# tjamescouch/abnn

Hardware: AMD Instinct MI355X
Metric: traversal events/sec at 1B synapses, 5M neurons; achieved HBM GB/s (higher is better)
Workload: dtype f32

## Files before the change

### abnn_amd/_lib.py

```python
from __future__ import annotations

import ctypes as C
import os

_HERE = os.path.dirname(os.path.abspath(__file__))
LIB_PATH = os.environ.get("ABNN_LIB") or os.path.join(_HERE, "libabnn_hip.so")

SUMMARY_WORDS = 4
COMM_ID_BYTES = 128


class Dims(C.Structure):

    _fields_ = [
        ("n_input", C.c_uint32),
        ("n_output", C.c_uint32),
        ("n_hidden", C.c_uint64),
        ("n_syn", C.c_uint64),
        ("events_per_pass", C.c_uint64),
        ("syn_offset", C.c_uint64),
        ("global_events", C.c_uint64),
        ("syn_capacity", C.c_uint64),
    ]

# ... 471 lines not shown
                   "abnn_reorder_host",
                   "abnn_propagate_words", "abnn_propagate_enqueue", "abnn_propagate", "abnn_propagate_rescale_enqueue",
                   "abnn_propagate_iterate_enqueue", "abnn_propagate_host", "abnn_propagate_rescale_host")

_lib = None


def _share_hip_runtime_with_torch() -> None:
    import importlib.util

    spec = importlib.util.find_spec("torch")
    if spec is None or not spec.submodule_search_locations:
        return
    hip = os.path.join(list(spec.submodule_search_locations)[0], "lib", "libamdhip64.so")
    if os.path.exists(hip):
        C.CDLL(hip, mode=C.RTLD_GLOBAL)


DEBUG_SIGNATURES = [
    ("abnn_debug_set_wave_clock", C.c_int, [_VP, C.c_int]),
    ("abnn_debug_raw_stats", C.c_int, [_VP, C.POINTER(C.c_uint64), _VP]),
    ("abnn_debug_raw_gate_timing", C.c_int, [C.c_int]),
    ("abnn_debug_raw_gate_time", C.c_int, [C.POINTER(C.c_double), _PU32]),
    ("abnn_debug_raw_fused", C.c_int, [C.c_int]),
    ("abnn_debug_raw_fused_active", C.c_int, []),
    ("abnn_debug_raw_wave_clock", C.c_int, [_VP, C.c_uint64, _U32, _U32, C.POINTER(C.c_uint64), C.c_uint64, _VP]),
    ("abnn_debug_live_allocations", C.c_uint64, []),
    ("abnn_debug_set_propagate_path", C.c_int, [_VP, C.c_int]),
    ("abnn_debug_index_state", C.c_int, [_VP, C.POINTER(C.c_uint64), C.POINTER(C.c_double)]),
    ("abnn_debug_index_mask_dirty", C.c_int, [_VP, C.POINTER(C.c_uint64)]),
    ("abnn_debug_set_indexed", C.c_int, [_VP, C.c_int]),
    ("abnn_debug_set_fused", C.c_int, [_VP, C.c_int]),
    ("abnn_debug_index_copy", C.c_int, [_VP, _PU32, C.c_uint64, _PU32, C.c_uint64]),
]


def load() -> C.CDLL:
    global _lib
    if _lib is not None:
        return _lib
    if not os.path.exists(LIB_PATH):
        raise ImportError(
            f"{LIB_PATH} not found: build it with `python -c 'import __graft_entry__ as g; g.build()'` "
            "(there is no CPU fallback for the traversal engine)")
    _share_hip_runtime_with_torch()
    lib = C.CDLL(LIB_PATH)
    for name, res, args in SIGNATURES + DEBUG_SIGNATURES:
        if not hasattr(lib, name) and ((name, res, args) in DEBUG_SIGNATURES or
                                       (os.environ.get("ABNN_LIB") and name in ABI10_ADDITIONS)):
            continue
        fn = getattr(lib, name)
        fn.restype = res
        fn.argtypes = args
    got = lib.abnn_abi_version()
    if got != ABI_VERSION:
        if not os.environ.get("ABNN_LIB_ANY_ABI"):
            raise ImportError(f"{LIB_PATH}: ABI version {got}, this binding is {ABI_VERSION} "
                              "(ABNN_LIB_ANY_ABI=1 accepts it for pass timing only)")
        import warnings

        warnings.warn(f"{LIB_PATH}: ABI version {got} != {ABI_VERSION}; use pass/timing entry points only")
    _lib = lib
    return lib


def check(fn_name: str, status: int) -> None:
# ... 24 lines not shown
```

### abnn_amd/csrc/capi.hip

```cpp
#include <dlfcn.h>
#include <link.h>
#include <rccl/rccl.h>

#include <algorithm>
#include <chrono>
#include <condition_variable>
#include <cstdio>
#include <cstdlib>
#include <cstring>
#include <mutex>
#include <new>
#include <string>
#include <vector>

#include "census.h"
#include "degree.h"
#include "select.h"
#include "edit.h"
#include "snapshot.h"
#include "graph.h"
#include "hops.h"
#include "engine.h"
#include "learn.h"
#include "spikes.h"
// ... 13 lines not shown
namespace {

#define HIP_TRY(expr)                                                                  \
    do {                                                                               \
        hipError_t _e = (expr);                                                        \
        if (_e != hipSuccess) {                                                        \
            set_err(std::string(#expr) + ": " + hipGetErrorString(_e));                \
            return ABNN_ERR_HIP;                                                       \
        }                                                                              \
    } while (0)

#define REQUIRE(cond, msg)                                                             \
    do {                                                                               \
        if (!(cond)) {                                                                 \
            set_err(msg);                                                              \
            return ABNN_ERR_INVALID;                                                   \
        }                                                                              \
    } while (0)

uint64_t visited_events(const abnn_dims& d, uint32_t mode)
{
    if (mode == ABNN_MODE_RANDOM) return d.n_syn ? d.events_per_pass : 0;
    uint64_t grid = (d.events_per_pass + 255u) / 256u * 256u;
    return grid < d.n_syn ? grid : d.n_syn;
}

struct EventPair {
    hipEvent_t a, b;
};

struct IndexState {
    uint32_t *row = nullptr, *off = nullptr, *mask = nullptr, *info = nullptr;
    uint4* heavy = nullptr;
    uint32_t heavy_chunks = 0;
    uint64_t mask_words = 0;
    bool built = false;
    uint64_t entries = 0;
    uint32_t max_degree = 0;
    float build_ms = 0.0f;
    uint64_t eligible = 0;
    bool last_indexed = false;
    uint64_t indexed_passes = 0;
    int flavour = -1;
    int mode = 1;
    uint32_t after = 4;
    uint64_t max_mb = 4096;
};

}

struct abnn_brain {
    abnn_dims dims{};
    abnn_params params{};
    KernelParams kp{};
    int device = 0;
    hipStream_t stream = nullptr;
    uint64_t n_nrn = 0;
    DevicePool pool;
    DeviceState d{};
    void* scalar_block = nullptr;
    uint64_t clock_host = 0;
    uint64_t rng = 0;
    uint64_t stim_first = 0, stim_count = 0;
    uint64_t clean_passes = 0, max_host_stamp = 0;
    uint64_t stim_ring[kFiredRing][2] = {};
    bool next_built = false;
// ... 210 lines not shown
void host_tick(abnn_brain* b)
{
    if (tick_events(b) > 0) b->clock_host += b->params.clock_inc;
}

abnn_status time_begin(abnn_brain* b, hipStream_t s, EventPair** out)
{
    *out = nullptr;
    if (b->timing <= 0) return ABNN_OK;
    const uint64_t n = (uint64_t)b->timing, c = b->timing_count++;
    if (c % n != (n > 1 ? 1u : 0u)) return ABNN_OK;
    if (b->events_used == b->events.size()) {
        EventPair p;
        HIP_TRY(hipEventCreate(&p.a));
        HIP_TRY(hipEventCreate(&p.b));
        b->events.push_back(p);
    }
    *out = &b->events[b->events_used++];
    HIP_TRY(hipEventRecord((*out)->a, s));
    return ABNN_OK;
}

constexpr uint64_t kStreamPinMiB = 160;
uint64_t stream_pin_bytes()
{
    uint64_t mib = kStreamPinMiB;
    if (const char* env = std::getenv("ABNN_STREAM_PIN_MB")) mib = (uint64_t)std::min(4096, std::max(0, std::atoi(env)));
    return mib << 20;
}

void index_invalidate(abnn_brain* b)
{
    IndexState& x = b->ix;
    if (x.row || x.off || x.mask || x.info || x.heavy) {
        (void)hipSetDevice(b->device);
        b->pool.release(&x.row, &x.off, &x.mask, &x.info, &x.heavy);
    }
    x.heavy_chunks = 0;
    x.built = false;
    x.entries = 0;
    x.max_degree = 0;
    x.mask_words = 0;
    x.eligible = 0;
}

void configure(abnn_brain* b)
{
    DeviceState& d = b->d;
    d.n_syn = b->dims.n_syn;
    const uint64_t ev = visited_events(b->dims, b->params.mode);
    if (ev != d.events) index_invalidate(b);
    d.events = ev;
    const uint64_t iters = (d.events + d.iter_events - 1) / d.iter_events;
    d.iters = (uint32_t)iters;
    uint64_t G = std::min<uint64_t>(iters, std::min<uint64_t>((uint64_t)b->cus * b->per_cu, kMaxGateBlocks));
    const uint64_t waves = d.gate_block / 64;
    G = std::min<uint64_t>(G, (iters + waves - 1) / waves);
    if (G == 0 && iters > 0) G = 1;
    d.gate_blocks = (uint32_t)G;
    d.n_ranges = (uint32_t)(G * waves);
    const uint64_t budget = stream_pin_bytes();
    d.pin_k = 0;
    if (d.events > 0 && b->params.mode == ABNN_MODE_SWEEP && !b->params.track_visits)
        d.pin_k = (uint32_t)std::min<uint64_t>(16, 16 * budget / (3 * d.events));
}

abnn_status reset_ranges(abnn_brain* b)
{
    const DeviceState& d = b->d;
    std::vector<uint32_t> rb(d.n_ranges + 1);
// ... 138 lines not shown
    d.stim_first = b->stim_first;
    d.stim_count = b->stim_count;
    const bool prebuilt = b->next_built && b->built_stim[0] == b->stim_first &&
                          b->built_stim[1] == b->stim_count;
    b->next_built = false;
    if (was_prebuilt) *was_prebuilt = prebuilt;
    if (!prebuilt) HIP_TRY(launch_bitmap(d, b->kp, b->stim_first, b->stim_count, s));
    b->stim_ring[b->pass_host % kFiredRing][0] = b->stim_first;
    b->stim_ring[b->pass_host % kFiredRing][1] = b->stim_count;
    return ABNN_OK;
}

void plan_build(abnn_brain* b)
{
    DeviceState& d = b->d;
    d.build_next = build_next_ok(b) ? 1u : 0u;
    d.n_next_stim = 0;
    if (d.build_next) {
        const uint64_t W = b->params.window_pre, p = b->pass_host;
        auto add = [&](uint64_t f, uint64_t c) {
            if (c == 0) return;
            for (uint32_t r = 0; r < d.n_next_stim; ++r)
                if (d.next_stim[r][0] == f && d.next_stim[r][1] == c) return;
            d.next_stim[d.n_next_stim][0] = f;
            d.next_stim[d.n_next_stim++][1] = c;
        };
        for (uint64_t q = p + 1 - W; q <= p; ++q) add(b->stim_ring[q % kFiredRing][0], b->stim_ring[q % kFiredRing][1]);
        add(b->stim_first, b->stim_count);
    }
}

uint64_t index_bytes(const abnn_brain* b)
{
    return 4 * b->d.events + 4 * (b->n_nrn + 1) + 4 * index_mask_words(b->d.iters, b->d.iter_events);
}

bool index_eligible(const abnn_brain* b)
{
    const DeviceState& d = b->d;
    const abnn_params& p = b->params;
    const bool plastic = p.w_prune > 0.0f || (d.grown != nullptr && p.p_new > 0.0f);
    return b->ix.mode != 0 && p.mode == ABNN_MODE_SWEEP && !p.track_visits && !plastic && d.lean && !d.g2src &&
           !b->ext_ptrs && b->dims.global_events == 0 && d.events > 0 && d.events < (1ull << 32) &&
           index_bytes(b) <= (b->ix.max_mb << 20);
}

bool index_pass_rule(const abnn_brain* b, bool prebuilt)
{
    if (!prebuilt) return false;
    const uint64_t W = b->params.window_pre, p = b->pass_host;
    uint64_t stim = b->stim_count;
    for (uint64_t q = p >= W ? p - W : 0; q <= p; ++q) stim = std::max(stim, b->stim_ring[q % kFiredRing][1]);
    const uint64_t bound = W * ((uint64_t)b->params.max_spikes + stim);
    return bound * b->ix.max_degree <= b->d.events / 8;
}

abnn_status index_build(abnn_brain* b, hipStream_t s)
{
    IndexState& x = b->ix;
    const DeviceState& d = b->d;
    index_invalidate(b);
    DeviceTemp<uint32_t> cursor, part;
    x.mask_words = index_mask_words(d.iters, d.iter_events);
    abnn_status st = b->pool.alloc_all({raw(&x.row, b->n_nrn + 1), raw(&x.off, d.events), zeroed(&x.mask, x.mask_words),
                                        zeroed(&x.info, 4)});
    if (st == ABNN_OK) st = cursor.alloc(b->n_nrn + 1, false);
    if (st == ABNN_OK) st = part.alloc(index_tiles(b->n_nrn) + 1, false);
    if (st != ABNN_OK) {
        index_invalidate(b);
        x.mode = 0;
        return st == ABNN_ERR_OOM ? ABNN_OK : st;
    }
    hipEvent_t ea = nullptr, eb = nullptr;
    HIP_TRY(hipEventCreate(&ea));
    hipError_t e = hipEventCreate(&eb);
    uint32_t info[4] = {0, 0, 0, 0};
    float ms = 0.0f;
    if (e == hipSuccess) e = hipEventRecord(ea, s);
    if (e == hipSuccess) e = launch_index_build(d.syn, d.events, b->n_nrn, x.row, cursor.dev, part.dev, x.off, x.info, (uint32_t)b->cus, s);
    if (e == hipSuccess) e = hipEventRecord(eb, s);
    if (e == hipSuccess) e = hipMemcpyAsync(info, x.info, sizeof(info), hipMemcpyDeviceToHost, s);
    if (e == hipSuccess) e = hipStreamSynchronize(s);
    if (e == hipSuccess) e = hipEventElapsedTime(&ms, ea, eb);
    (void)hipEventDestroy(ea);
    if (eb) (void)hipEventDestroy(eb);
    HIP_TRY(e);
    x.max_degree = info[0];
    x.entries = info[1];
    x.build_ms = ms;
    if (info[2]) {
        st = b->pool.alloc(raw(&x.heavy, info[2]));
        if (st != ABNN_OK) {
            index_invalidate(b);
            x.mode = 0;
            return st == ABNN_ERR_OOM ? ABNN_OK : st;
        }
        HIP_TRY(launch_index_heavy(x.row, b->n_nrn, x.heavy, info[2], x.info, s));
    }
// ... 43 lines not shown
        b->next_built = d.build_next != 0;
        b->built_stim[0] = b->stim_first;
        b->built_stim[1] = b->stim_count;
        rotate_bounds(b);
        return ABNN_OK;
    }
    plan_build(b);
    HIP_TRY(launch_apply(d, b->kp, gathered, world, rank, s));
    b->next_built = d.build_next != 0;
    b->built_stim[0] = b->stim_first;
    b->built_stim[1] = b->stim_count;
    rotate_bounds(b);
    return ABNN_OK;
}

abnn_status run_fused(abnn_brain* b, hipStream_t s)
{
    DeviceState& d = b->d;
    IndexState& x = b->ix;
    const bool eligible = index_eligible(b);
    if (eligible && !x.built && x.eligible >= x.after) ST_TRY(index_build(b, s));
    bool prebuilt = false;
    ST_TRY(pass_buffers(b, s, &prebuilt));
    plan_build(b);
    const bool indexed = eligible && x.built && (x.mode == 2 || index_pass_rule(b, prebuilt));
    d.prologue_adapt = b->last_pass_fused && x.flavour == (indexed ? 1 : 0) && d.adapt_ranges ? 1u : 0u;
    d.cost_in = b->cost_buf[b->cost_parity ^ 1u];
    d.cost_out = b->cost_buf[b->cost_parity];
    d.indexed = indexed ? 1u : 0u;
    d.ev_mask = x.mask;
    EventPair* ev = nullptr;
    ST_TRY(time_begin(b, s, &ev));
    hipError_t e = hipSuccess;
    if (indexed)
        e = launch_index_mark(d.bitmap, d.n_bitmap_words, d.n_nrn, x.row, x.off, x.mask, d.events, x.heavy, x.heavy_chunks, s);
    if (e == hipSuccess) e = launch_fused_pass(d, b->kp, s);
    d.indexed = 0u;
    HIP_TRY(e);
    if (ev) HIP_TRY(hipEventRecord(ev->b, s));
    x.flavour = indexed ? 1 : 0;
    x.last_indexed = indexed;
    x.indexed_passes += indexed ? 1u : 0u;
    x.eligible = eligible ? x.eligible + 1 : 0;
    b->next_built = d.build_next != 0;
    b->built_stim[0] = b->stim_first;
    b->built_stim[1] = b->stim_count;
    rotate_bounds(b);
    b->cost_parity ^= 1u;
    b->last_pass_fused = true;
    return ABNN_OK;
}

abnn_status run_shard_fused_gate(abnn_brain* b, int32_t* xchg, hipStream_t s)
{
    DeviceState& d = b->d;
    ST_TRY(pass_buffers(b, s));
    plan_build(b);
    d.prologue_adapt = b->last_pass_fused && d.adapt_ranges ? 1u : 0u;
    d.cost_in = b->cost_buf[b->cost_parity ^ 1u];
    d.cost_out = b->cost_buf[b->cost_parity];
    d.shard_mode = 1;
    d.xchg = xchg;
    b->ix.eligible = 0;
    b->ix.last_indexed = false;
    b->ix.flavour = 0;
    EventPair* ev = nullptr;
    ST_TRY(time_begin(b, s, &ev));
    const hipError_t e = launch_fused_pass(d, b->kp, s);
// ... 1979 lines not shown
    ST_TRY(sync_all(b));
    HIP_TRY(hipMemcpy(out, b->d.range_bounds, std::min<uint64_t>(n, b->d.n_ranges + 1ull) * 4, hipMemcpyDeviceToHost));
    return ABNN_OK;
}

abnn_status abnn_debug_stream_pin(abnn_brain* b, uint32_t* pin_k)
{
    REQUIRE(b && pin_k, "null argument");
    *pin_k = b->d.pin_k;
    return ABNN_OK;
}

abnn_status abnn_debug_index_state(abnn_brain* b, uint64_t out[ABNN_DEBUG_INDEX_WORDS], double* build_ms)
{
    REQUIRE(b && out, "null argument");
    const IndexState& x = b->ix;
    out[0] = x.built ? 1 : 0;
    out[1] = x.entries;
    out[2] = x.max_degree;
    out[3] = x.last_indexed ? 1 : 0;
    out[4] = x.indexed_passes;
    out[5] = x.eligible;
    out[6] = (uint64_t)x.mode;
    out[7] = b->d.events;
    if (build_ms) *build_ms = x.build_ms;
    return ABNN_OK;
}

abnn_status abnn_debug_index_mask_dirty(abnn_brain* b, uint64_t* words)
{
    REQUIRE(b && words, "null argument");
    *words = 0;
    ST_TRY(sync_all(b));
    if (!b->ix.mask) return ABNN_OK;
    HIP_TRY(launch_index_dirty(b->ix.mask, b->ix.mask_words, reinterpret_cast<unsigned long long*>(b->u64_scratch), b->stream));
    return read_words(b, b->u64_scratch, words, 1);
}

abnn_status abnn_debug_set_indexed(abnn_brain* b, int mode)
{
    REQUIRE(b && mode >= 0 && mode <= 2, "abnn_debug_set_indexed: mode must be 0, 1 or 2");
    b->ix.mode = mode;
    return ABNN_OK;
}

abnn_status abnn_debug_set_fused(abnn_brain* b, int on)
{
    REQUIRE(b, "null argument");
    REQUIRE(!b->pending_walk, "abnn_debug_set_fused: a sharded pass is half done (abnn_shard_apply)");
    b->use_fused = on != 0;
    return ABNN_OK;
}

abnn_status abnn_debug_index_copy(abnn_brain* b, uint32_t* row, uint64_t n_row, uint32_t* off, uint64_t n_off)
{
    REQUIRE(b && (row || n_row == 0) && (off || n_off == 0), "null argument");
    ST_TRY(sync_all(b));
    REQUIRE(b->ix.built, "abnn_debug_index_copy: no index is built");
    REQUIRE(n_row <= b->n_nrn + 1 && n_off <= b->ix.entries, "abnn_debug_index_copy: range out of bounds");
    if (n_row) HIP_TRY(hipMemcpy(row, b->ix.row, n_row * 4, hipMemcpyDeviceToHost));
    if (n_off) HIP_TRY(hipMemcpy(off, b->ix.off, n_off * 4, hipMemcpyDeviceToHost));
    return ABNN_OK;
}

uint64_t abnn_debug_live_allocations(void) { return g_live_allocations.load(std::memory_order_relaxed); }

abnn_status abnn_get_stats(abnn_brain* b, abnn_stats* out)
{
    REQUIRE(b && out, "null argument");
// ... 545 lines not shown
```

### abnn_amd/csrc/engine.h

```cpp
#pragma once

#include <hip/hip_runtime.h>
#include <cstdint>

#include "../../include/abnn/abnn.h"

namespace abnn {

constexpr int kMaxFilterWords = 16384;
constexpr uint32_t kF2Words = 2048;
__host__ __device__ inline uint32_t f2_hash1(uint32_t n) { return (n * 0x9E3779B1u) >> 16; }
__host__ __device__ inline uint32_t f2_hash2(uint32_t n) { return (n * 0x85EBCA77u + 0x165667B1u) >> 16; }
constexpr int kScanThreads = 1024;
constexpr int kMaxGateBlocks = 1024;
constexpr int kMaxRanges = 16384;
constexpr int kApplyThreads = 1024;
constexpr uint32_t kCandCap = 256;
constexpr uint32_t kFusedMaxRanges = 4096;
constexpr uint32_t kWalkBlocks = 256;
constexpr int kMaxApplyBlocks = kWalkBlocks;
static_assert(kMaxApplyBlocks <= kApplyThreads, "the finalizing workgroup reads one apply partial per thread");
static_assert(kMaxRanges % kApplyThreads == 0, "range prefix: whole ranges per thread");
constexpr int kDummyRecords = 64 * 32;
constexpr uint32_t kFiredRing = 8;
// ... 95 lines not shown
    uint32_t chunk_penalty;
    uint32_t apply_blocks;
    uint32_t range_map;
    uint32_t pin_k;
    uint64_t* lb_status;
    const uint32_t* cost_in;
    uint32_t* cost_out;
    uint2* cand_list;
    uint32_t flush_at;
    int32_t spec_margin;
    uint32_t spec_mode;
    uint32_t lean;
    uint32_t shard_mode;
    int32_t* xchg;
    uint32_t prologue_adapt;
    uint64_t n_syn;
    uint64_t n_nrn;
    uint32_t n_input;
    uint64_t events;
    uint64_t syn_offset;
    uint64_t seed;
    uint32_t mode;
    uint32_t n_bitmap_words;
    uint32_t filter_words;
    uint32_t filter_log2;
    uint32_t gate_blocks;
    uint32_t n_ranges;
    uint32_t iters;
    uint32_t iter_events;
    uint32_t gate_block;
    uint32_t gate_k;
    uint32_t fused_max_blocks;
    uint32_t indexed;
    uint32_t* ev_mask;
};

struct KernelParams {
    float base_scale, target_rate_hz, eta_home, eta_reward, alpha_rbar;
    float a_ltp, a_ltd, w_min, w_max;
    uint32_t refractory, window_pre, clock_inc, max_spikes;
    uint32_t track_visits;
    float w_prune, p_new, w_init;
    uint32_t compact_every;
};

__host__ __device__ constexpr uint32_t xchg_words(uint32_t max_spikes)
{
    return 2 * ABNN_SUMMARY_WORDS + ((max_spikes + 1u) & ~1u);
}

constexpr int kCompactThreads = 1024;
constexpr int kCompactChunk = 4 * kCompactThreads;

KernelParams to_kernel_params(const abnn_params& p);

bool gate_shape_supported(uint32_t block, uint32_t k, uint32_t filter_words);
int gate_blocks_per_cu(uint32_t block, uint32_t k, uint32_t filter_words, bool track, bool random);

hipError_t launch_bitmap(const DeviceState& d, const KernelParams& kp, uint64_t stim_first,
                         uint64_t stim_count, hipStream_t s);
hipError_t launch_gate(const DeviceState& d, const KernelParams& kp, hipStream_t s);
bool fused_pass_supported(const DeviceState& d);
int fused_blocks_per_cu(uint32_t block, uint32_t k, uint32_t filter_words, bool track);
hipError_t launch_fused_pass(const DeviceState& d, const KernelParams& kp, hipStream_t s);
hipError_t launch_shard_walk(const DeviceState& d, const KernelParams& kp, const int32_t* gathered, uint32_t world,
                             uint32_t rank, hipStream_t s);
hipError_t launch_scan(const DeviceState& d, const KernelParams& kp, int32_t* xchg_out, hipStream_t s);
// ... 22 lines not shown
```

### abnn_amd/csrc/index.h

```cpp
#pragma once

#include "engine.h"

namespace abnn {

constexpr uint32_t kMaskRoundBytes = 4096;
inline uint64_t index_mask_words(uint64_t iters, uint64_t iter_events)
{
    return iters * iter_events / 32 + 2 * kMaskRoundBytes / 4;
}

constexpr uint32_t kIndexTile = 4096;
inline uint64_t index_tiles(uint64_t n_nrn) { return (n_nrn + kIndexTile - 1) / kIndexTile; }

hipError_t launch_index_build(const SynArrays& syn, uint64_t events, uint64_t n_nrn, uint32_t* row, uint32_t* cursor,
                              uint32_t* part, uint32_t* off, uint32_t* info, uint32_t cus, hipStream_t s);
hipError_t launch_index_heavy(const uint32_t* row, uint64_t n_nrn, uint4* heavy, uint32_t chunks, uint32_t* info,
                              hipStream_t s);
hipError_t launch_index_mark(const uint32_t* bitmap, uint32_t n_words, uint64_t n_nrn, const uint32_t* row,
                             const uint32_t* off, uint32_t* mask, uint64_t events, const uint4* heavy, uint32_t chunks,
                             hipStream_t s);
hipError_t launch_index_dirty(const uint32_t* mask, uint64_t words, unsigned long long* out, hipStream_t s);

}
```

### abnn_amd/csrc/index.hip

```cpp
#include "index.h"
#include "runs.h"
#include "scan.h"
#include "device.h"

namespace abnn {
namespace {

constexpr uint32_t kHeavyLen = 128, kHeavyChunk = 1024;

__device__ __forceinline__ void wave_lds_sync()
{
    __builtin_amdgcn_fence(__ATOMIC_RELEASE, "wavefront", "local");
    __builtin_amdgcn_wave_barrier();
    __builtin_amdgcn_fence(__ATOMIC_ACQUIRE, "wavefront", "local");
}

struct SrcPair {
    uint32_t k0, k1;
};

__device__ __forceinline__ SrcPair load_src_pair(const SynArrays& a, uint64_t base, uint32_t lane, uint64_t events,
                                                 uint32_t n_nrn)
{
    const uint64_t p = (base >> 1) + lane;
// ... 83 lines not shown
    }
    uint32_t total;
    uint32_t ex = part[blockIdx.x] + block_scan_u32(sum, &total, s_wave);
#pragma unroll
    for (uint32_t j = 0; j < 4; ++j) {
        if (i0 + j < n_nrn) {
            row[i0 + j] = ex;
            cursor[i0 + j] = ex;
        }
        ex += c[j];
    }
    if (blockIdx.x == 0 && threadIdx.x == 0) row[n_nrn] = part[tiles];
}

__global__ __launch_bounds__(256) void k_index_scatter(SynArrays a, uint64_t events, uint32_t n_nrn, uint32_t* cursor,
                                                       uint32_t* off)
{
    const uint32_t lane = threadIdx.x & 63;
    const uint64_t wave = ((uint64_t)blockIdx.x * 256 + threadIdx.x) >> 6, waves = (uint64_t)gridDim.x * 4;
    for (uint64_t base = wave * 128; base < events; base += waves * 128) {
        const SrcPair k = load_src_pair(a, base, lane, events, n_nrn);
        const uint64_t e0 = base + 2 * lane;
        if (k.k0 != kRunNone) {
            const uint32_t q = atomicAdd(cursor + k.k0, 1u);
            if (q < events) off[q] = (uint32_t)e0;
        }
        if (k.k1 != kRunNone) {
            const uint32_t q = atomicAdd(cursor + k.k1, 1u);
            if (q < events) off[q] = (uint32_t)(e0 + 1);
        }
    }
}

__device__ __forceinline__ void wave_mask_or(uint32_t* mask, bool act, uint32_t o)
{
    constexpr int kMerge = 8;
    const uint32_t lane = threadIdx.x & 63, w = o >> 5, bit = 1u << (o & 31u);
    for (int it = 0; it < kMerge; ++it) {
        const uint64_t m = __ballot(act);
        if (m == 0) return;
        const uint32_t lead = (uint32_t)__builtin_ctzll(m);
        const uint32_t wl = (uint32_t)__builtin_amdgcn_readlane((int)w, (int)lead);
        const bool same = act && w == wl;
        if (__popcll(__ballot(same)) == 1) break;
        uint32_t bits = same ? bit : 0u;
#pragma unroll
        for (int x = 32; x > 0; x >>= 1) bits |= __shfl_xor(bits, x, 64);
        if (lane == lead) (void)__hip_atomic_fetch_or(mask + wl, bits, __ATOMIC_RELAXED, __HIP_MEMORY_SCOPE_AGENT);
        act = act && !same;
    }
    if (act) (void)__hip_atomic_fetch_or(mask + w, bit, __ATOMIC_RELAXED, __HIP_MEMORY_SCOPE_AGENT);
}

constexpr uint32_t kMarkWaves = 4, kMarkWords = 16, kMarkBatch = 256;

__global__ __launch_bounds__(kMarkWaves * 64) void k_index_mark(const uint32_t* bitmap, uint32_t n_words, uint32_t n_nrn,
                                                                const uint32_t* row, const uint32_t* off, uint32_t* mask,
                                                                uint64_t events, const uint4* heavy, uint32_t light)
{
    __shared__ uint16_t s_n[kMarkWaves][kMarkWords * 32];
    __shared__ uint32_t s_beg[kMarkWaves][kMarkBatch], s_pre[kMarkWaves][kMarkBatch];
    const uint32_t lane = threadIdx.x & 63, wid = wave_uniform(threadIdx.x >> 6);
    if (blockIdx.x >= light) {
        const uint4 it = heavy[blockIdx.x - light];
        if (((bitmap[it.x >> 5] >> (it.x & 31u)) & 1u) == 0u) return;
        uint32_t o[4];
#pragma unroll
        for (uint32_t u = 0; u < 4; ++u) {
            const uint32_t j = (u * kMarkWaves + wid) * 64 + lane;
            o[u] = j < it.z ? off[it.y + j] : 0xFFFFFFFFu;
        }
#pragma unroll
        for (uint32_t u = 0; u < 4; ++u) wave_mask_or(mask, o[u] < events, o[u]);
        return;
    }
    const uint32_t w0 = (blockIdx.x * kMarkWaves + wid) * kMarkWords;
    if (w0 >= n_words) return;
    const uint32_t word = lane < kMarkWords && w0 + lane < n_words ? bitmap[w0 + lane] : 0u;
    const uint32_t cnt = (uint32_t)__builtin_popcount(word), inc = wave_incl_scan(cnt);
    const uint32_t total = (uint32_t)__builtin_amdgcn_readlane((int)inc, 63);
    if (total == 0) return;
    uint32_t q = inc - cnt;
    for (uint32_t m = word; m; m &= m - 1u) s_n[wid][q++] = (uint16_t)(lane * 32u + (uint32_t)__builtin_ctz(m));
    wave_lds_sync();
    for (uint32_t c0 = 0; c0 < total; c0 += kMarkBatch) {
        uint32_t b[4], len[4];
#pragma unroll
        for (uint32_t u = 0; u < 4; ++u) {
            const uint32_t i = c0 + u * 64 + lane;
            const uint32_t n = i < total ? w0 * 32u + s_n[wid][i] : 0xFFFFFFFFu;
            const bool vn = n < n_nrn;
            const uint32_t e = vn ? row[n + 1] : 0u;
            b[u] = vn ? row[n] : 0u;
            len[u] = e > b[u] && e - b[u] <= kHeavyLen ? e - b[u] : 0u;
        }
        uint32_t T = 0;
#pragma unroll
        for (uint32_t u = 0; u < 4; ++u) {
            const uint32_t pre = wave_incl_scan(len[u]);
            s_beg[wid][u * 64 + lane] = b[u];
            s_pre[wid][u * 64 + lane] = T + pre - len[u];
            T += (uint32_t)__builtin_amdgcn_readlane((int)pre, 63);
        }
        wave_lds_sync();
        for (uint32_t j0 = 0; j0 < T; j0 += 256) {
            uint32_t o[4];
#pragma unroll
            for (uint32_t u = 0; u < 4; ++u) {
                const uint32_t j = j0 + u * 64 + lane;
                uint32_t lo = 0, hi = kMarkBatch;
#pragma unroll
                for (int st = 0; st < 8; ++st) {
                    const uint32_t mid = (lo + hi) >> 1;
                    if (s_pre[wid][mid] <= j) lo = mid;
                    else hi = mid;
                }
                o[u] = j < T ? off[s_beg[wid][lo] + (j - s_pre[wid][lo])] : 0xFFFFFFFFu;
            }
#pragma unroll
            for (uint32_t u = 0; u < 4; ++u) wave_mask_or(mask, o[u] < events, o[u]);
        }
        wave_lds_sync();
    }
}

__global__ __launch_bounds__(256) void k_index_heavy_fill(const uint32_t* row, uint32_t n_nrn, uint4* heavy, uint32_t cap,
                                                          uint32_t* cursor)
{
    const uint64_t n = (uint64_t)blockIdx.x * 256 + threadIdx.x;
    if (n >= n_nrn) return;
    const uint32_t b = row[n], len = row[n + 1] - b;
    if (len <= kHeavyLen) return;
    const uint32_t nch = (len + kHeavyChunk - 1) / kHeavyChunk, slot = atomicAdd(cursor, nch);
    for (uint32_t c = 0; c < nch && slot + c < cap; ++c)
        heavy[slot + c] = make_uint4((uint32_t)n, b + c * kHeavyChunk, min(kHeavyChunk, len - c * kHeavyChunk), 0u);
}

__global__ __launch_bounds__(256) void k_index_dirty(const uint32_t* mask, uint64_t words, unsigned long long* out)
{
    uint32_t n = 0;
    for (uint64_t i = (uint64_t)blockIdx.x * 256 + threadIdx.x; i < words; i += (uint64_t)gridDim.x * 256) n += mask[i] != 0u;
    n = wave_add(n);
    if ((threadIdx.x & 63) == 0 && n) atomicAdd(out, (unsigned long long)n);
}

}

hipError_t launch_index_build(const SynArrays& syn, uint64_t events, uint64_t n_nrn, uint32_t* row, uint32_t* cursor,
                              uint32_t* part, uint32_t* off, uint32_t* info, uint32_t cus, hipStream_t s)
{
    const uint32_t tiles = (uint32_t)index_tiles(n_nrn), nn = (uint32_t)n_nrn;
    hipError_t e = hipMemsetAsync(cursor, 0, (n_nrn + 1) * 4, s);
    if (e == hipSuccess) e = hipMemsetAsync(info, 0, 4 * 4, s);
    if (e != hipSuccess) return e;
    const uint64_t steps = (events + 511) / 512;
    const uint32_t grid = (uint32_t)std::max<uint64_t>(1, std::min<uint64_t>((uint64_t)std::max(1u, cus) * 8, steps));
    hipLaunchKernelGGL(k_index_count, dim3(grid), dim3(256), 0, s, syn, events, nn, cursor);
    hipLaunchKernelGGL(k_index_scan_a, dim3(tiles), dim3(1024), 0, s, cursor, nn, part, info);
    hipLaunchKernelGGL(k_index_scan_b, dim3(1), dim3(1024), 0, s, part, tiles, info);
    hipLaunchKernelGGL(k_index_scan_c, dim3(tiles), dim3(1024), 0, s, cursor, nn, part, tiles, row);
    hipLaunchKernelGGL(k_index_scatter, dim3(grid), dim3(256), 0, s, syn, events, nn, cursor, off);
    return hipGetLastError();
}

hipError_t launch_index_heavy(const uint32_t* row, uint64_t n_nrn, uint4* heavy, uint32_t chunks, uint32_t* info,
                              hipStream_t s)
{
    if (chunks == 0 || n_nrn == 0) return hipSuccess;
    hipLaunchKernelGGL(k_index_heavy_fill, dim3((uint32_t)((n_nrn + 255) / 256)), dim3(256), 0, s, row, (uint32_t)n_nrn, heavy,
                       chunks, info + 3);
    return hipGetLastError();
}

hipError_t launch_index_mark(const uint32_t* bitmap, uint32_t n_words, uint64_t n_nrn, const uint32_t* row,
                             const uint32_t* off, uint32_t* mask, uint64_t events, const uint4* heavy, uint32_t chunks,
                             hipStream_t s)
{
    if (n_words == 0) return hipSuccess;
    const uint32_t per = kMarkWaves * kMarkWords, light = (n_words + per - 1) / per;
    hipLaunchKernelGGL(k_index_mark, dim3(light + chunks), dim3(kMarkWaves * 64), 0, s, bitmap, n_words, (uint32_t)n_nrn, row,
                       off, mask, events, heavy, light);
    return hipGetLastError();
}

hipError_t launch_index_dirty(const uint32_t* mask, uint64_t words, unsigned long long* out, hipStream_t s)
{
    hipError_t e = hipMemsetAsync(out, 0, 8, s);
    if (e != hipSuccess) return e;
    const uint32_t grid = (uint32_t)std::max<uint64_t>(1, std::min<uint64_t>(2048, (words + 255) / 256));
    hipLaunchKernelGGL(k_index_dirty, dim3(grid), dim3(256), 0, s, mask, words, out);
    return hipGetLastError();
}

}
```

### abnn_amd/csrc/kernels.hip

```cpp
#include <algorithm>
#include <type_traits>

#include "engine.h"
#include "device.h"
#include "index.h"

#pragma clang fp contract(off)

namespace abnn {

KernelParams to_kernel_params(const abnn_params& p)
{
    KernelParams k;
    k.base_scale = p.base_scale;
    k.target_rate_hz = p.target_rate_hz;
    k.eta_home = p.eta_home;
    k.eta_reward = p.eta_reward;
    k.alpha_rbar = p.alpha_rbar;
    k.a_ltp = p.a_ltp;
    k.a_ltd = p.a_ltd;
    k.w_min = p.w_min;
    k.w_max = p.w_max;
    k.refractory = p.refractory;
    k.window_pre = p.window_pre;
// ... 1052 lines not shown
                asm volatile("; pinned");
#pragma unroll
                for (int b = 0; b < NB8; ++b) {
                    x.lo[b] = bl[b * 64 + lane];
                    x.hi[b] = bh[b * 64 + lane];
                }
                asm volatile("; pinned end");
            } else {
#pragma unroll
                for (int b = 0; b < NB8; ++b) {
                    x.lo[b] = __builtin_nontemporal_load(bl + b * 64 + lane);
                    x.hi[b] = __builtin_nontemporal_load(bh + b * 64 + lane);
                }
            }
            if constexpr (kTrack) {
                const u32x4* bd = reinterpret_cast<const u32x4*>(live ? reinterpret_cast<const uint32_t*>(d.syn.dw + (uint64_t)it * IE)
                                                                      : d.dummy);
#pragma unroll
                for (int b = 0; b < NB8; ++b)
#pragma unroll
                    for (int j = 0; j < 4; ++j) {
                        const u32x4 v = __builtin_nontemporal_load(bd + b * 256 + lane * 4 + j);
                        x.dd[8 * b + 2 * j] = v.x;
                        x.dd[8 * b + 2 * j + 1] = v.z;
                    }
            }
        }
    };
    constexpr uint32_t BI = IE / 8, RI = kMaskRoundBytes / BI;
    constexpr int ML = kMaskRoundBytes / 1024;
    static_assert(!kMask || (size_t)FW * sizeof(uint2) >= (size_t)NW * kMaskRoundBytes, "the mask rounds fit the filter's LDS");
    u32x4 mk[ML];
    u32x4* const mrow = reinterpret_cast<u32x4*>(s_fb) + wid * (kMaskRoundBytes / 16);
    auto mask_at = [&](uint32_t it0) { return reinterpret_cast<u32x4*>(d.ev_mask) + (uint64_t)it0 * (BI / 16); };
    auto mask_issue = [&](uint32_t it0) __attribute__((always_inline)) {
        const u32x4* p = mask_at(it0);
#pragma unroll
        for (int j = 0; j < ML; ++j) mk[j] = p[j * 64 + lane];
    };
    __builtin_amdgcn_sched_barrier(0);
    if constexpr (kMask) {
        mask_issue(it_begin);
    } else {
#pragma unroll
    for (int j = 0; j < kDepth; ++j) issue(bufs[j], it_begin + j, it_begin + j < it_end);
    }
    if constexpr (!kFused) {
        zero_next_images(d, FW, BLOCK, now);
        lds_barrier();
    } else {
        if (tid < 5) s_fz.stat[tid] = 0u;
        if (tid == 0) s_fz.done = 0u;
        if (tid == 0) s_fz.sg2 = 0u;
        if (tid < kSetCache) s_fz.setc[tid] = ~0ull;
        constexpr int kRecLoads = kMask ? ML : kDepth * (kRandom ? K * (kTrack ? 2 : 1) : NB8 * (2 + (kTrack ? 4 : 0)));
        __builtin_amdgcn_sched_barrier(0);
        wait_vm_lgkm0<kRecLoads>();
        __builtin_amdgcn_s_barrier();
        __builtin_amdgcn_fence(__ATOMIC_ACQUIRE, "workgroup", "local");
    }
    const uint64_t t_start = __builtin_amdgcn_s_memrealtime();
    uint64_t* wcb = d.wave_clock + (kFused ? (pass_f % kWaveClockPasses) * (uint64_t)kWaveClock * kMaxRanges : 0);
    if (lane == 0 && d.wave_clock_on) {
        wcb[kWaveClock * r] = t_start;
        wcb[kWaveClock * r + 3] = t_entry;
    }
    const uint64_t len = it_end - it_begin;
// ... 170 lines not shown
                    uint32_t q = pend + P - p0;
                    do {
                        if ((x0 | x1) != 0u) {
                            const bool hs = x0 == 0u;
                            const uint32_t xx = hs ? x1 : x0, m = (uint32_t)__builtin_ctz(xx) >> 3;
                            const uint32_t xn = xx & (xx - 1u);
                            x0 = hs ? x0 : xn;
                            x1 = hs ? xn : x1;
                            const uint32_t e0 = hs ? w2 : w0, e1 = hs ? w3 : w1;
                            const uint32_t lo16 = __builtin_amdgcn_perm(e1, e0, 0x0C0C0100u + m * 0x0202u);
                            st_off[q] = relb + (hs ? 4u : 0u) + m;
                            st_src[q] = __builtin_amdgcn_perm(hs ? v1 : v0, lo16, 0x0C040100u + (m << 16));
                            ++q;
                        }
                    } while (__ballot((x0 | x1) != 0u) != 0);
                    pend += p1 - p0;
                    if (kFused ? pend >= d.flush_at : pend >= kChunk) {
                        if constexpr (kFused) flush_all();
                        else chunk_out();
                    }
                }
            }
        }
    };
    if constexpr (kMask) {
        (void)step;
        const uint8_t* mbytes = reinterpret_cast<const uint8_t*>(mrow);
        constexpr uint32_t PI = 1024 / BI;
        for (uint32_t r0 = it_begin; r0 < it_end; r0 += RI) {
            u32x4 cur[ML];
#pragma unroll
            for (int j = 0; j < ML; ++j) cur[j] = mk[j];
            if (r0 + RI < it_end) mask_issue(r0 + RI);
            u32x4* const mp = mask_at(r0);
#pragma unroll
            for (int j = 0; j < ML; ++j) {
                const bool in = r0 + (uint32_t)(j * 1024 + lane * 16) / BI < it_end;
                if (!in) cur[j] = u32x4{0u, 0u, 0u, 0u};
                if ((cur[j].x | cur[j].y | cur[j].z | cur[j].w) != 0u) mp[j * 64 + lane] = u32x4{0u, 0u, 0u, 0u};
                mrow[j * 64 + lane] = cur[j];
            }
            __builtin_amdgcn_fence(__ATOMIC_RELEASE, "wavefront", "local");
            __builtin_amdgcn_wave_barrier();
            __builtin_amdgcn_fence(__ATOMIC_ACQUIRE, "wavefront", "local");
#pragma unroll 1
            for (uint32_t j = 0; j < (uint32_t)ML; ++j) {
                if (r0 + j * PI >= it_end) break;
                const u32x4 v = mrow[j * 64 + lane];
                const uint32_t w4[4] = {v.x, v.y, v.z, v.w};
                const uint32_t c = __builtin_popcount(w4[0]) + __builtin_popcount(w4[1]) + __builtin_popcount(w4[2]) +
                                   __builtin_popcount(w4[3]);
                const uint32_t inc = wave_incl_scan(c);
                const uint32_t hits = (uint32_t)__builtin_amdgcn_readlane((int)inc, 63);
                if (hits == 0) continue;
                const uint32_t rel0 = (uint32_t)((uint64_t)(r0 + j * PI) * IE - region);
                if (pend + hits <= SE) {
                    uint32_t q = pend + inc - c;
#pragma unroll
                    for (int w = 0; w < 4; ++w)
                        for (uint32_t x = w4[w]; x != 0u; x &= x - 1u)
                            st_off[q++] = rel0 + 128u * lane + 32u * w + (uint32_t)__builtin_ctz(x);
                    pend += hits;
                    if (pend >= d.flush_at) flush_all();
                    continue;
                }
#pragma unroll 1
                for (uint32_t b = 0; b < 1024 / 64; ++b) {
                    const uint32_t byte = mbytes[1024u * j + 64u * b + lane];
                    const uint64_t bb = __ballot(byte != 0u);
                    if (bb == 0) continue;
                    const uint32_t relb = rel0 + 512u * b + 8u * lane;
                    const uint32_t cb = __builtin_popcount(byte);
// ... 1194 lines not shown
```

### include/abnn/abnn_debug.h

```cpp
#ifndef ABNN_ABNN_DEBUG_H
#define ABNN_ABNN_DEBUG_H

#include "abnn.h"

#ifdef __cplusplus
extern "C" {
#endif

abnn_status abnn_debug_set_wave_clock(abnn_brain* b, int on);
abnn_status abnn_debug_wave_clock(abnn_brain* b, uint64_t* out, uint64_t n);
abnn_status abnn_debug_wave_clock_slot(abnn_brain* b, uint32_t slot, uint64_t* out, uint64_t n);
abnn_status abnn_debug_apply_clock(abnn_brain* b, uint64_t* out, uint64_t n);
abnn_status abnn_debug_bitmap(abnn_brain* b, uint32_t* out, uint64_t n, int* incremental_next);
abnn_status abnn_debug_range_bounds(abnn_brain* b, uint32_t* out, uint64_t n);
abnn_status abnn_debug_stream_pin(abnn_brain* b, uint32_t* pin_k);

abnn_status abnn_debug_raw_stats(const void* workspace, uint64_t* out2, void* stream);
abnn_status abnn_debug_raw_gate_timing(int enable);
abnn_status abnn_debug_raw_gate_time(double* total_ms, uint32_t* launches);
abnn_status abnn_debug_raw_fused(int mode);
int abnn_debug_raw_fused_active(void);
abnn_status abnn_debug_raw_wave_clock(const void* workspace, uint64_t workspace_bytes, uint32_t n_syn,
                                      uint32_t events, uint64_t* out, uint64_t n, void* stream);

abnn_status abnn_debug_comm_allgather(abnn_comm* c, void* buf, uint64_t bytes, uint32_t count, void* stream);

uint64_t abnn_debug_live_allocations(void);

abnn_status abnn_debug_set_propagate_path(abnn_brain* b, int path);

#define ABNN_DEBUG_INDEX_WORDS 8
abnn_status abnn_debug_index_state(abnn_brain* b, uint64_t out[ABNN_DEBUG_INDEX_WORDS], double* build_ms);
abnn_status abnn_debug_index_mask_dirty(abnn_brain* b, uint64_t* words);
abnn_status abnn_debug_set_indexed(abnn_brain* b, int mode);
abnn_status abnn_debug_set_fused(abnn_brain* b, int on);
abnn_status abnn_debug_index_copy(abnn_brain* b, uint32_t* row, uint64_t n_row, uint32_t* off, uint64_t n_off);

#ifdef __cplusplus
}
#endif
#endif
```

Before: 2771 billion.

## Maintain index event mask incrementally from fired-neuron bitmap deltas

```diff
diff --git a/abnn_amd/_lib.py b/abnn_amd/_lib.py
--- a/abnn_amd/_lib.py
+++ b/abnn_amd/_lib.py
@@ -527,6 +527,8 @@
     ("abnn_debug_set_indexed", C.c_int, [_VP, C.c_int]),
     ("abnn_debug_set_fused", C.c_int, [_VP, C.c_int]),
     ("abnn_debug_index_copy", C.c_int, [_VP, _PU32, C.c_uint64, _PU32, C.c_uint64]),
+    ("abnn_debug_index_mask_copy", C.c_int, [_VP, _PU32, C.c_uint64, _PU32, C.c_uint64]),
+    ("abnn_debug_index_delta", C.c_int, [_VP, C.POINTER(C.c_uint64)]),
 ]
 
 
diff --git a/abnn_amd/csrc/capi.hip b/abnn_amd/csrc/capi.hip
--- a/abnn_amd/csrc/capi.hip
+++ b/abnn_amd/csrc/capi.hip
@@ -69,6 +69,8 @@
 struct IndexState {
     uint32_t *row = nullptr, *off = nullptr, *mask = nullptr, *info = nullptr;
     uint4* heavy = nullptr;
+    uint32_t *marked = nullptr, *marked_next = nullptr, *delta = nullptr;
+    uint32_t delta_at = 0;
     uint32_t heavy_chunks = 0;
     uint64_t mask_words = 0;
     bool built = false;
@@ -345,10 +347,11 @@
 void index_invalidate(abnn_brain* b)
 {
     IndexState& x = b->ix;
-    if (x.row || x.off || x.mask || x.info || x.heavy) {
+    if (x.row || x.off || x.mask || x.info || x.heavy || x.marked || x.marked_next || x.delta) {
         (void)hipSetDevice(b->device);
-        b->pool.release(&x.row, &x.off, &x.mask, &x.info, &x.heavy);
-    }
+        b->pool.release(&x.row, &x.off, &x.mask, &x.info, &x.heavy, &x.marked, &x.marked_next, &x.delta);
+    }
+    x.delta_at = 0;
     x.heavy_chunks = 0;
     x.built = false;
     x.entries = 0;
@@ -553,7 +556,8 @@
 
 uint64_t index_bytes(const abnn_brain* b)
 {
-    return 4 * b->d.events + 4 * (b->n_nrn + 1) + 4 * index_mask_words(b->d.iters, b->d.iter_events);
+    return 4 * b->d.events + 4 * (b->n_nrn + 1) + 4 * index_mask_words(b->d.iters, b->d.iter_events) +
+           2 * 4 * (uint64_t)b->d.n_bitmap_words + 2 * 4 * 4 * (uint64_t)kDeltaSlots + 4 * 4;
 }
 
 bool index_eligible(const abnn_brain* b)
@@ -584,7 +588,8 @@
     DeviceTemp<uint32_t> cursor, part;
     x.mask_words = index_mask_words(d.iters, d.iter_events);
     abnn_status st = b->pool.alloc_all({raw(&x.row, b->n_nrn + 1), raw(&x.off, d.events), zeroed(&x.mask, x.mask_words),
-                                        zeroed(&x.info, 4)});
+                                        zeroed(&x.info, 4), zeroed(&x.marked, d.n_bitmap_words),
+                                        zeroed(&x.marked_next, d.n_bitmap_words), zeroed(&x.delta, 2 * 4 * kDeltaSlots)});
     if (st == ABNN_OK) st = cursor.alloc(b->n_nrn + 1, false);
     if (st == ABNN_OK) st = part.alloc(index_tiles(b->n_nrn) + 1, false);
     if (st != ABNN_OK) {
@@ -694,8 +699,15 @@
     EventPair* ev = nullptr;
     ST_TRY(time_begin(b, s, &ev));
     hipError_t e = hipSuccess;
-    if (indexed)
-        e = launch_index_mark(d.bitmap, d.n_bitmap_words, d.n_nrn, x.row, x.off, x.mask, d.events, x.heavy, x.heavy_chunks, s);
+    if (indexed) {
+        const uint32_t at = x.delta_at ^ 4u * kDeltaSlots;
+        e = launch_index_mark(d.bitmap, x.marked, x.marked_next, d.n_bitmap_words, d.n_nrn, x.row, x.off, x.mask, d.events,
+                              x.heavy, x.heavy_chunks, x.delta + at, x.delta + x.delta_at, s);
+        if (e == hipSuccess) {
+            std::swap(x.marked, x.marked_next);
+            x.delta_at = at;
+        }
+    }
     if (e == hipSuccess) e = launch_fused_pass(d, b->kp, s);
     d.indexed = 0u;
     HIP_TRY(e);
@@ -2741,9 +2753,42 @@
     REQUIRE(b && words, "null argument");
     *words = 0;
     ST_TRY(sync_all(b));
-    if (!b->ix.mask) return ABNN_OK;
-    HIP_TRY(launch_index_dirty(b->ix.mask, b->ix.mask_words, reinterpret_cast<unsigned long long*>(b->u64_scratch), b->stream));
+    const IndexState& x = b->ix;
+    if (!x.mask) return ABNN_OK;
+    const DeviceState& d = b->d;
+    DeviceTemp<uint32_t> want, none, next;
+    ST_TRY(want.alloc(x.mask_words));
+    ST_TRY(none.alloc(d.n_bitmap_words));
+    ST_TRY(next.alloc(d.n_bitmap_words, false));
+    if (x.built)
+        HIP_TRY(launch_index_mark(x.marked, none.dev, next.dev, d.n_bitmap_words, d.n_nrn, x.row, x.off, want.dev, d.events,
+                                  x.heavy, x.heavy_chunks, nullptr, nullptr, b->stream));
+    HIP_TRY(launch_index_dirty(x.mask, want.dev, x.mask_words, reinterpret_cast<unsigned long long*>(b->u64_scratch), b->stream));
     return read_words(b, b->u64_scratch, words, 1);
+}
+
+abnn_status abnn_debug_index_mask_copy(abnn_brain* b, uint32_t* mask_words_out, uint64_t n_words, uint32_t* marked_out,
+                                       uint64_t n_marked_words)
+{
+    REQUIRE(b && (mask_words_out || n_words == 0) && (marked_out || n_marked_words == 0), "null argument");
+    ST_TRY(sync_all(b));
+    REQUIRE(b->ix.built, "abnn_debug_index_mask_copy: no index is built");
+    n_words = std::min<uint64_t>(n_words, b->ix.mask_words);
+    n_marked_words = std::min<uint64_t>(n_marked_words, b->d.n_bitmap_words);
+    if (n_words) HIP_TRY(hipMemcpy(mask_words_out, b->ix.mask, n_words * 4, hipMemcpyDeviceToHost));
+    if (n_marked_words) HIP_TRY(hipMemcpy(marked_out, b->ix.marked, n_marked_words * 4, hipMemcpyDeviceToHost));
+    return ABNN_OK;
+}
+
+abnn_status abnn_debug_index_delta(abnn_brain* b, uint64_t out[4])
+{
+    REQUIRE(b && out, "null argument");
+    ST_TRY(sync_all(b));
+    std::vector<uint32_t> v(4 * kDeltaSlots, 0u);
+    if (b->ix.delta) HIP_TRY(hipMemcpy(v.data(), b->ix.delta + b->ix.delta_at, v.size() * 4, hipMemcpyDeviceToHost));
+    for (int i = 0; i < 4; ++i) out[i] = 0;
+    for (size_t i = 0; i < v.size(); ++i) out[i & 3] += v[i];
+    return ABNN_OK;
 }
 
 abnn_status abnn_debug_set_indexed(abnn_brain* b, int mode)
diff --git a/abnn_amd/csrc/engine.h b/abnn_amd/csrc/engine.h
--- a/abnn_amd/csrc/engine.h
+++ b/abnn_amd/csrc/engine.h
@@ -151,7 +151,7 @@
     uint32_t gate_k;
     uint32_t fused_max_blocks;
     uint32_t indexed;
-    uint32_t* ev_mask;
+    const uint32_t* ev_mask;
 };
 
 struct KernelParams {
diff --git a/abnn_amd/csrc/index.h b/abnn_amd/csrc/index.h
--- a/abnn_amd/csrc/index.h
+++ b/abnn_amd/csrc/index.h
@@ -17,9 +17,11 @@
                               uint32_t* part, uint32_t* off, uint32_t* info, uint32_t cus, hipStream_t s);
 hipError_t launch_index_heavy(const uint32_t* row, uint64_t n_nrn, uint4* heavy, uint32_t chunks, uint32_t* info,
                               hipStream_t s);
-hipError_t launch_index_mark(const uint32_t* bitmap, uint32_t n_words, uint64_t n_nrn, const uint32_t* row,
-                             const uint32_t* off, uint32_t* mask, uint64_t events, const uint4* heavy, uint32_t chunks,
-                             hipStream_t s);
-hipError_t launch_index_dirty(const uint32_t* mask, uint64_t words, unsigned long long* out, hipStream_t s);
+constexpr uint32_t kDeltaSlots = 1024;
+hipError_t launch_index_mark(const uint32_t* bitmap, const uint32_t* marked, uint32_t* marked_next, uint32_t n_words,
+                             uint64_t n_nrn, const uint32_t* row, const uint32_t* off, uint32_t* mask, uint64_t events,
+                             const uint4* heavy, uint32_t chunks, uint32_t* delta, uint32_t* delta_next, hipStream_t s);
+hipError_t launch_index_dirty(const uint32_t* mask, const uint32_t* want, uint64_t words, unsigned long long* out,
+                              hipStream_t s);
 
 }
diff --git a/abnn_amd/csrc/index.hip b/abnn_amd/csrc/index.hip
--- a/abnn_amd/csrc/index.hip
+++ b/abnn_amd/csrc/index.hip
@@ -139,9 +139,14 @@
     }
 }
 
-__device__ __forceinline__ void wave_mask_or(uint32_t* mask, bool act, uint32_t o)
+template <bool kClear>
+__device__ __forceinline__ void wave_mask_apply(uint32_t* mask, bool act, uint32_t o)
 {
     constexpr int kMerge = 8;
+    auto apply = [&](uint32_t word, uint32_t bits) {
+        if constexpr (kClear) (void)__hip_atomic_fetch_and(mask + word, ~bits, __ATOMIC_RELAXED, __HIP_MEMORY_SCOPE_AGENT);
+        else (void)__hip_atomic_fetch_or(mask + word, bits, __ATOMIC_RELAXED, __HIP_MEMORY_SCOPE_AGENT);
+    };
     const uint32_t lane = threadIdx.x & 63, w = o >> 5, bit = 1u << (o & 31u);
     for (int it = 0; it < kMerge; ++it) {
         const uint64_t m = __ballot(act);
@@ -153,24 +158,39 @@
         uint32_t bits = same ? bit : 0u;
 #pragma unroll
         for (int x = 32; x > 0; x >>= 1) bits |= __shfl_xor(bits, x, 64);
-        if (lane == lead) (void)__hip_atomic_fetch_or(mask + wl, bits, __ATOMIC_RELAXED, __HIP_MEMORY_SCOPE_AGENT);
+        if (lane == lead) apply(wl, bits);
         act = act && !same;
     }
-    if (act) (void)__hip_atomic_fetch_or(mask + w, bit, __ATOMIC_RELAXED, __HIP_MEMORY_SCOPE_AGENT);
+    if (act) apply(w, bit);
+}
+
+__device__ __forceinline__ void wave_mask_delta(uint32_t* mask, uint64_t events, uint32_t o, bool leave)
+{
+    const bool valid = o < events;
+    wave_mask_apply<false>(mask, valid && !leave, o);
+    wave_mask_apply<true>(mask, valid && leave, o);
 }
 
 constexpr uint32_t kMarkWaves = 4, kMarkWords = 16, kMarkBatch = 256;
 
-__global__ __launch_bounds__(kMarkWaves * 64) void k_index_mark(const uint32_t* bitmap, uint32_t n_words, uint32_t n_nrn,
-                                                                const uint32_t* row, const uint32_t* off, uint32_t* mask,
-                                                                uint64_t events, const uint4* heavy, uint32_t light)
+__global__ __launch_bounds__(kMarkWaves * 64) void k_index_mark(const uint32_t* now, const uint32_t* old, uint32_t* next,
+                                                                uint32_t n_words, uint32_t n_nrn, const uint32_t* row,
+                                                                const uint32_t* off, uint32_t* mask, uint64_t events,
+                                                                const uint4* heavy, uint32_t light, uint32_t* delta,
+                                                                uint32_t* delta_next)
 {
     __shared__ uint16_t s_n[kMarkWaves][kMarkWords * 32];
     __shared__ uint32_t s_beg[kMarkWaves][kMarkBatch], s_pre[kMarkWaves][kMarkBatch];
     const uint32_t lane = threadIdx.x & 63, wid = wave_uniform(threadIdx.x >> 6);
+    if (delta_next)
+        for (uint32_t i = blockIdx.x * (kMarkWaves * 64) + threadIdx.x; i < 4 * kDeltaSlots; i += gridDim.x * (kMarkWaves * 64))
+            delta_next[i] = 0u;
+    if (delta) delta += 4u * ((blockIdx.x * kMarkWaves + wid) & (kDeltaSlots - 1u));
     if (blockIdx.x >= light) {
         const uint4 it = heavy[blockIdx.x - light];
-        if (((bitmap[it.x >> 5] >> (it.x & 31u)) & 1u) == 0u) return;
+        const uint32_t was = (old[it.x >> 5] >> (it.x & 31u)) & 1u, is = (now[it.x >> 5] >> (it.x & 31u)) & 1u;
+        if (was == is) return;
+        const bool leave = was != 0u;
         uint32_t o[4];
 #pragma unroll
         for (uint32_t u = 0; u < 4; ++u) {
@@ -178,18 +198,27 @@
             o[u] = j < it.z ? off[it.y + j] : 0xFFFFFFFFu;
         }
 #pragma unroll
-        for (uint32_t u = 0; u < 4; ++u) wave_mask_or(mask, o[u] < events, o[u]);
+        for (uint32_t u = 0; u < 4; ++u) wave_mask_delta(mask, events, o[u], leave);
+        if (delta && threadIdx.x == 0) atomicAdd(delta + (leave ? 3 : 2), it.z);
         return;
     }
     const uint32_t w0 = (blockIdx.x * kMarkWaves + wid) * kMarkWords;
     if (w0 >= n_words) return;
-    const uint32_t word = lane < kMarkWords && w0 + lane < n_words ? bitmap[w0 + lane] : 0u;
-    const uint32_t cnt = (uint32_t)__builtin_popcount(word), inc = wave_incl_scan(cnt);
-    const uint32_t total = (uint32_t)__builtin_amdgcn_readlane((int)inc, 63);
-    if (total == 0) return;
-    uint32_t q = inc - cnt;
-    for (uint32_t m = word; m; m &= m - 1u) s_n[wid][q++] = (uint16_t)(lane * 32u + (uint32_t)__builtin_ctz(m));
+    const bool mine = lane < kMarkWords && w0 + lane < n_words;
+    const uint32_t wnow = mine ? now[w0 + lane] : 0u, wold = mine ? old[w0 + lane] : 0u;
+    if (mine) next[w0 + lane] = wnow;
+    if (__ballot(wnow != wold) == 0) return;
+    const uint32_t went = wnow & ~wold, wlev = wold & ~wnow;
+    const uint32_t ce = (uint32_t)__builtin_popcount(went), ie = wave_incl_scan(ce);
+    const uint32_t cl = (uint32_t)__builtin_popcount(wlev), il = wave_incl_scan(cl);
+    const uint32_t n_ent = (uint32_t)__builtin_amdgcn_readlane((int)ie, 63);
+    const uint32_t total = n_ent + (uint32_t)__builtin_amdgcn_readlane((int)il, 63);
+    uint32_t q = ie - ce;
+    for (uint32_t m = went; m; m &= m - 1u) s_n[wid][q++] = (uint16_t)(lane * 32u + (uint32_t)__builtin_ctz(m));
+    q = n_ent + il - cl;
+    for (uint32_t m = wlev; m; m &= m - 1u) s_n[wid][q++] = (uint16_t)(lane * 32u + (uint32_t)__builtin_ctz(m));
     wave_lds_sync();
+    uint32_t set = 0, clr = 0;
     for (uint32_t c0 = 0; c0 < total; c0 += kMarkBatch) {
         uint32_t b[4], len[4];
 #pragma unroll
@@ -200,6 +229,8 @@
             const uint32_t e = vn ? row[n + 1] : 0u;
             b[u] = vn ? row[n] : 0u;
             len[u] = e > b[u] && e - b[u] <= kHeavyLen ? e - b[u] : 0u;
+            set += i < n_ent ? len[u] : 0u;
+            clr += i < n_ent ? 0u : len[u];
         }
         uint32_t T = 0;
 #pragma unroll
@@ -212,6 +243,7 @@
         wave_lds_sync();
         for (uint32_t j0 = 0; j0 < T; j0 += 256) {
             uint32_t o[4];
+            bool leave[4];
 #pragma unroll
             for (uint32_t u = 0; u < 4; ++u) {
                 const uint32_t j = j0 + u * 64 + lane;
@@ -223,11 +255,18 @@
                     else hi = mid;
                 }
                 o[u] = j < T ? off[s_beg[wid][lo] + (j - s_pre[wid][lo])] : 0xFFFFFFFFu;
+                leave[u] = c0 + lo >= n_ent;
             }
 #pragma unroll
-            for (uint32_t u = 0; u < 4; ++u) wave_mask_or(mask, o[u] < events, o[u]);
+            for (uint32_t u = 0; u < 4; ++u) wave_mask_delta(mask, events, o[u], leave[u]);
         }
         wave_lds_sync();
+    }
+    if (delta) {
+        set = wave_add(set);
+        clr = wave_add(clr);
+        const uint32_t v = lane == 0 ? n_ent : lane == 1 ? total - n_ent : lane == 2 ? set : clr;
+        if (lane < 4 && v) atomicAdd(delta + lane, v);
     }
 }
 
@@ -243,10 +282,11 @@
         heavy[slot + c] = make_uint4((uint32_t)n, b + c * kHeavyChunk, min(kHeavyChunk, len - c * kHeavyChunk), 0u);
 }
 
-__global__ __launch_bounds__(256) void k_index_dirty(const uint32_t* mask, uint64_t words, unsigned long long* out)
+__global__ __launch_bounds__(256) void k_index_dirty(const uint32_t* mask, const uint32_t* want, uint64_t words,
+                                                     unsigned long long* out)
 {
     uint32_t n = 0;
-    for (uint64_t i = (uint64_t)blockIdx.x * 256 + threadIdx.x; i < words; i += (uint64_t)gridDim.x * 256) n += mask[i] != 0u;
+    for (uint64_t i = (uint64_t)blockIdx.x * 256 + threadIdx.x; i < words; i += (uint64_t)gridDim.x * 256) n += mask[i] != want[i];
     n = wave_add(n);
     if ((threadIdx.x & 63) == 0 && n) atomicAdd(out, (unsigned long long)n);
 }
@@ -279,23 +319,24 @@
     return hipGetLastError();
 }
 
-hipError_t launch_index_mark(const uint32_t* bitmap, uint32_t n_words, uint64_t n_nrn, const uint32_t* row,
-                             const uint32_t* off, uint32_t* mask, uint64_t events, const uint4* heavy, uint32_t chunks,
-                             hipStream_t s)
+hipError_t launch_index_mark(const uint32_t* bitmap, const uint32_t* marked, uint32_t* marked_next, uint32_t n_words,
+                             uint64_t n_nrn, const uint32_t* row, const uint32_t* off, uint32_t* mask, uint64_t events,
+                             const uint4* heavy, uint32_t chunks, uint32_t* delta, uint32_t* delta_next, hipStream_t s)
 {
     if (n_words == 0) return hipSuccess;
     const uint32_t per = kMarkWaves * kMarkWords, light = (n_words + per - 1) / per;
-    hipLaunchKernelGGL(k_index_mark, dim3(light + chunks), dim3(kMarkWaves * 64), 0, s, bitmap, n_words, (uint32_t)n_nrn, row,
-                       off, mask, events, heavy, light);
+    hipLaunchKernelGGL(k_index_mark, dim3(light + chunks), dim3(kMarkWaves * 64), 0, s, bitmap, marked, marked_next, n_words,
+                       (uint32_t)n_nrn, row, off, mask, events, heavy, light, delta, delta_next);
     return hipGetLastError();
 }
 
-hipError_t launch_index_dirty(const uint32_t* mask, uint64_t words, unsigned long long* out, hipStream_t s)
+hipError_t launch_index_dirty(const uint32_t* mask, const uint32_t* want, uint64_t words, unsigned long long* out,
+                              hipStream_t s)
 {
     hipError_t e = hipMemsetAsync(out, 0, 8, s);
     if (e != hipSuccess) return e;
     const uint32_t grid = (uint32_t)std::max<uint64_t>(1, std::min<uint64_t>(2048, (words + 255) / 256));
-    hipLaunchKernelGGL(k_index_dirty, dim3(grid), dim3(256), 0, s, mask, words, out);
+    hipLaunchKernelGGL(k_index_dirty, dim3(grid), dim3(256), 0, s, mask, want, words, out);
     return hipGetLastError();
 }
 
diff --git a/abnn_amd/csrc/kernels.hip b/abnn_amd/csrc/kernels.hip
--- a/abnn_amd/csrc/kernels.hip
+++ b/abnn_amd/csrc/kernels.hip
@@ -1108,7 +1108,7 @@
     static_assert(!kMask || (size_t)FW * sizeof(uint2) >= (size_t)NW * kMaskRoundBytes, "the mask rounds fit the filter's LDS");
     u32x4 mk[ML];
     u32x4* const mrow = reinterpret_cast<u32x4*>(s_fb) + wid * (kMaskRoundBytes / 16);
-    auto mask_at = [&](uint32_t it0) { return reinterpret_cast<u32x4*>(d.ev_mask) + (uint64_t)it0 * (BI / 16); };
+    auto mask_at = [&](uint32_t it0) { return reinterpret_cast<const u32x4*>(d.ev_mask) + (uint64_t)it0 * (BI / 16); };
     auto mask_issue = [&](uint32_t it0) __attribute__((always_inline)) {
         const u32x4* p = mask_at(it0);
 #pragma unroll
@@ -1345,12 +1345,10 @@
 #pragma unroll
             for (int j = 0; j < ML; ++j) cur[j] = mk[j];
             if (r0 + RI < it_end) mask_issue(r0 + RI);
-            u32x4* const mp = mask_at(r0);
 #pragma unroll
             for (int j = 0; j < ML; ++j) {
                 const bool in = r0 + (uint32_t)(j * 1024 + lane * 16) / BI < it_end;
                 if (!in) cur[j] = u32x4{0u, 0u, 0u, 0u};
-                if ((cur[j].x | cur[j].y | cur[j].z | cur[j].w) != 0u) mp[j * 64 + lane] = u32x4{0u, 0u, 0u, 0u};
                 mrow[j * 64 + lane] = cur[j];
             }
             __builtin_amdgcn_fence(__ATOMIC_RELEASE, "wavefront", "local");
diff --git a/include/abnn/abnn_debug.h b/include/abnn/abnn_debug.h
--- a/include/abnn/abnn_debug.h
+++ b/include/abnn/abnn_debug.h
@@ -32,6 +32,9 @@
 #define ABNN_DEBUG_INDEX_WORDS 8
 abnn_status abnn_debug_index_state(abnn_brain* b, uint64_t out[ABNN_DEBUG_INDEX_WORDS], double* build_ms);
 abnn_status abnn_debug_index_mask_dirty(abnn_brain* b, uint64_t* words);
+abnn_status abnn_debug_index_mask_copy(abnn_brain* b, uint32_t* mask_words_out, uint64_t n_words, uint32_t* marked_out,
+                                       uint64_t n_marked_words);
+abnn_status abnn_debug_index_delta(abnn_brain* b, uint64_t out[4]);
 abnn_status abnn_debug_set_indexed(abnn_brain* b, int mode);
 abnn_status abnn_debug_set_fused(abnn_brain* b, int on);
 abnn_status abnn_debug_index_copy(abnn_brain* b, uint32_t* row, uint64_t n_row, uint32_t* off, uint64_t n_off);
```

Measured after the change: 3366 billion (median of 6 runs). 1.21x the previous value.
